# jw007123/hp-Adaptive-Signed-Distance-Field-Octree

Hardware: AMD Instinct MI355X
Metric: Query() Mpts/sec at targetError=1e-5 (union3 field, 10M SplitMix64 pts per GPU, HBM-resident); Create() ms reported as create_ms (higher is better)
Workload: dtype f64

## Files before the change

### hp-adaptive-signed-distance-field-octree_amd/csrc/field_eval.hpp

```cpp
#pragma once
#include <hip/hip_runtime.h>

#include "device_types.hpp"

namespace hpsdf {

template <bool LEFT>
__device__ __forceinline__ double sum3(double a, double b, double c) {
    if constexpr (LEFT) return (a + b) + c;
    else return a + (b + c);
}
template <bool LEFT>
__device__ __forceinline__ double prod3(double a, double b, double c) {
    if constexpr (LEFT) return (a * b) * c;
    else return a * (b * c);
}
__device__ __forceinline__ double sqrtExact(double x) {
    const uint32_t hi = (uint32_t)__double2hiint(x);
    const bool plain = hi - 0x10000000u < 0x7FF00000u - 0x10000000u;
    if (__builtin_amdgcn_ballot_w64(!plain) != 0ull) return sqrt(x);
    const double y = __builtin_amdgcn_rsq(x);
    double g = x * y, h = y * 0.5;
    const double r = __builtin_fma(-h, g, 0.5);
    g = __builtin_fma(g, r, g);
    h = __builtin_fma(h, r, h);
    double d = __builtin_fma(-g, g, x);
    g = __builtin_fma(d, h, g);
    d = __builtin_fma(-g, g, x);
    return __builtin_fma(d, h, g);
}

template <bool LEFT>
__device__ __forceinline__ double norm3(double x, double y, double z) { return sqrtExact(sum3<LEFT>(x * x, y * y, z * z)); }

template <bool LEFT>
__device__ __forceinline__ double primEval(const hpsdf_prim& pr, double x, double y, double z) {
    const double* p = pr.p;
    switch (pr.kind) {
        case HPSDF_PRIM_SPHERE:
            return norm3<LEFT>(x - p[0], y - p[1], z - p[2]) - p[3];
        case HPSDF_PRIM_BOX: {
            const double qx = fabs(x - p[0]) - p[3];
            const double qy = fabs(y - p[1]) - p[4];
            const double qz = fabs(z - p[2]) - p[5];
            const double outside = norm3<LEFT>(fmax(qx, 0.0), fmax(qy, 0.0), fmax(qz, 0.0));
            const double inside = fmin(fmax(qx, fmax(qy, qz)), 0.0);
            return outside + inside;
        }
        case HPSDF_PRIM_TORUS_Y: {
            const double dx = x - p[0], dy = y - p[1], dz = z - p[2];
            const double l = sqrtExact(dx * dx + dz * dz) - p[3];
            return sqrtExact(l * l + dy * dy) - p[4];
        }
        case HPSDF_PRIM_PLANE:
            return (p[0] * x + (p[1] * y + p[2] * z)) + p[3];
        default:
            return 0.0;
    }
}

template <bool LEFT>
__device__ __forceinline__ double analyticEval(const FieldDev& f, double x, double y, double z) {
    double acc = primEval<LEFT>(f.prims[0], x, y, z);
    for (int i = 1; i < f.nPrims; ++i) {
        const double d = primEval<LEFT>(f.prims[i], x, y, z);
        switch (f.prims[i].op) {
            case HPSDF_OP_UNION: acc = fmin(acc, d); break;
            case HPSDF_OP_INTERSECT: acc = fmax(acc, d); break;
            default: acc = fmax(acc, -d); break;
        }
    }
    return acc;
}

}
```

### hp-adaptive-signed-distance-field-octree_amd/csrc/fit_kernels.hpp

```cpp
#pragma once
#include <hip/hip_runtime.h>

#include <cstdint>

#include "device_types.hpp"
#include "field_glue.hpp"
#include "launch.hpp"

namespace hpsdf {


constexpr int kFitPiece = 8;
#ifndef HPSDF_FIT_MIN_WAVES
#define HPSDF_FIT_MIN_WAVES 4
#endif

__device__ __forceinline__ double fitRowAny(double acc, double a1, const double* __restrict__ tk, double n2,
                                            const double* __restrict__ F, int nq) {
    int k = 0;
    for (; k + 4 <= nq; k += 4) {
        const double f0 = F[k], f1 = F[k + 1], f2 = F[k + 2], f3 = F[k + 3];
        const double t0 = tk[k], t1 = tk[k + 1], t2 = tk[k + 2], t3 = tk[k + 3];
        acc = acc + (a1 * t0 * n2) * f0;
        acc = acc + (a1 * t1 * n2) * f1;
        acc = acc + (a1 * t2 * n2) * f2;
        acc = acc + (a1 * t3 * n2) * f3;
    }
    for (; k < nq; ++k) acc = acc + (a1 * tk[k] * n2) * F[k];
    return acc;
}

template <int KIND, bool CSG, int DEG, int R, bool LEFT>
__device__ __forceinline__ void fitBlockBody(const FitBlock blk, const FitTask* __restrict__ tasks, double* __restrict__ arena,
                                             double* __restrict__ errs, double* __restrict__ mirror,
                                             const DeviceTables* __restrict__ T, const FieldDev& field, const RootMap& rm, double* lds) {
    static_assert(R == 1 || DEG > 0, "cell blocking needs a compile-time degree");
    __shared__ double sNl[13 * 11];
    __shared__ double sRec[26];
    __shared__ int32_t sMeshStack[kFitThreads / 64][kMeshStack];
    __shared__ unsigned char sPosI[KIND == kFieldMesh ? 64 : 4], sPosJK[KIND == kFieldMesh ? 64 : 4];
    const int tid = threadIdx.x;
    const int deg = DEG > 0 ? DEG : (int)blk.degree;
    const int nq = 4 * deg + 1, nq2 = nq * nq, G = blk.nTasks;
    const int rowStart = blk.rowStart, rowEnd = blk.rowEnd, nrows = rowEnd - rowStart;
    const int gl = nq * (nq - 1) / 2;
    const int planes = blk.planesPerChunk;
    const int depth = blk.depth;
    const bool split = blk.split != 0;

    double* sT = lds;
    double* sR = sT + (deg + 1) * nq;
    double* sW = sR + nq;
    double* sC = sW + nq;
    double* sF = sC + 8 * G;

    stageQueryTables(T, sNl, sRec);
    for (int q = tid; q < nq; q += kFitThreads) {
        const double x = T->roots[gl + q];
        sR[q] = x;
        sW[q] = T->weights[gl + q];
        double m2 = 0.0, m1 = 1.0;
        sT[q] = 1.0;
        for (int i = 1; i <= deg; ++i) {
            const double l = T->rec[i][0] * x * m1 - T->rec[i][1] * m2;
            m2 = m1, m1 = l;
            sT[i * nq + q] = l;
        }
    }
    for (int g = tid; g < G; g += kFitThreads) {
        const FitTask& tk = tasks[blk.firstTask + g];
        double sc[3];
        for (int a = 0; a < 3; ++a) {
            sc[a] = (double)(tk.bmax[a] - tk.bmin[a]) * 0.5;
            sC[8 * g + 3 + a] = (double)((tk.bmin[a] + tk.bmax[a]) / 2.0f);
            sC[8 * g + a] = sc[a];
        }
        sC[8 * g + 6] = prod3<LEFT>(sc[0], sc[1], sc[2]);
        sC[8 * g + 7] = __longlong_as_double((long long)tk.sampleOff);
    }
    __syncthreads();

    const bool wide = DEG == 0 && nrows > kFitThreads;
    const int slot = wide ? 0 : tid / nrows;
    const int g2 = slot * R;
    const int r0 = rowStart + (wide ? tid : tid % nrows);
    const int r1 = r0 + kFitThreads;
    const bool act0 = wide ? (r0 < rowEnd) : (tid < ((G + R - 1) / R) * nrows);
    const bool act1 = wide && r1 < rowEnd;
    int i0a = 0, i1a = 0, i2a = 0, i0b = 0, i1b = 0, i2b = 0;
    double n0a = 0, n1a = 0, n2a = 0, n0b = 0, n1b = 0, n2b = 0;
    if (act0) {
        i0a = T->bidx[r0][0], i1a = T->bidx[r0][1], i2a = T->bidx[r0][2];
        n0a = sNl[i0a * 11 + depth], n1a = sNl[i1a * 11 + depth], n2a = sNl[i2a * 11 + depth];
    }
    if (act1) {
        i0b = T->bidx[r1][0], i1b = T->bidx[r1][1], i2b = T->bidx[r1][2];
        n0b = sNl[i0b * 11 + depth], n1b = sNl[i1b * 11 + depth], n2b = sNl[i2b * 11 + depth];
    }
    constexpr int NQF = DEG > 0 ? 4 * DEG + 1 : 1;
    double tkReg[NQF];
    if (DEG > 0) {
#pragma unroll
        for (int k = 0; k < NQF; ++k) tkReg[k] = sT[i2a * nq + k];
    }
    uint32_t meshHint = 0xFFFFFFFFu;
    double acc[R];
#pragma unroll
    for (int r = 0; r < R; ++r) acc[r] = 0.0;
    double acc1 = 0.0;

    const int cellStride = planes * nq2;
    for (int iBase = 0; iBase < nq; iBase += planes) {
        const int np = min(planes, nq - iBase);
        if constexpr (KIND == kFieldMesh) {
            if (tid < nq) {
                int rank = 0;
                for (int b = 0; b < nq; ++b) rank += sR[b] < sR[tid] ? 1 : 0;
                sPosJK[rank] = (unsigned char)tid;
            }
            if (tid >= 64 && tid < 64 + np) {
                const int a = tid - 64;
                int rank = 0;
                for (int b = 0; b < np; ++b) rank += sR[iBase + b] < sR[iBase + a] ? 1 : 0;
                sPosI[rank] = (unsigned char)a;
            }
            __syncthreads();
        }
        if constexpr (KIND != kFieldMesh) {
            const int cols = G * nq2;
            for (int c0 = 0; c0 < cols; c0 += kFitThreads) {
                const int cc = c0 + tid;
                const bool activeS = cc < cols;
                const int ccl = activeS ? cc : cols - 1;
                const int g = ccl / nq2, jk = ccl - g * nq2, j = jk / nq, k = jk - j * nq;
                const double* c = sC + 8 * g;
                const double uy = sR[j] * c[1] + c[4], uz = sR[k] * c[2] + c[5];
                const double wy = uy * rm.bounds[1] + rm.centre[1];
                const double wz = uz * rm.bounds[2] + rm.centre[2];
                const double wj = sW[j], wk = sW[k], c6 = c[6];
                const uint64_t sbase = (uint64_t)__double_as_longlong(c[7]) + (uint64_t)(j * nq + k);
                for (int il = 0; il < np; ++il) {
                    const int i = iBase + il;
                    const double ux = sR[i] * c[0] + c[3];
                    const double wx = ux * rm.bounds[0] + rm.centre[0];
                    const uint64_t sidx = sbase + (uint64_t)(i * nq2);
                    const double fv = activeS ? fieldEvalWorld<KIND, CSG, LEFT>(field, wx, wy, wz, sidx, sNl, sRec, meshHint) : 0.0;
                    if (activeS) {
                        sF[g * cellStride + il * nq2 + jk] = c6 * prod3<LEFT>(sW[i], wj, wk) * fv;
                        if (split) const_cast<double*>(field.samples)[sidx] = fv;
                    }
                }
            }
        } else {
            const int chunkSamples = np * nq2, total = G * chunkSamples;
            const float invChunk = 1.0f / (float)chunkSamples;
            for (int s0 = 0; s0 < total; s0 += kFitThreads) {
                const int s = s0 + tid;
                const bool activeS = s < total;
                const int sc = activeS ? s : total - 1;
                int g = (int)(((float)sc + 0.5f) * invChunk);
                int rem = sc - g * chunkSamples;
                if (rem < 0) {
                    --g;
                    rem += chunkSamples;
                } else if (rem >= chunkSamples) {
                    ++g;
                    rem -= chunkSamples;
                }
                if constexpr (KIND == kFieldMesh) rem = meshSampleOrder(rem, np, nq, sPosI, sPosJK);
                const double* c = sC + 8 * g;
                const int il = rem / nq2, jk = rem - il * nq2, j = jk / nq, k = jk - j * nq, i = iBase + il;
                const double ux = sR[i] * c[0] + c[3], uy = sR[j] * c[1] + c[4], uz = sR[k] * c[2] + c[5];
                const double wx = ux * rm.bounds[0] + rm.centre[0];
                const double wy = uy * rm.bounds[1] + rm.centre[1];
                const double wz = uz * rm.bounds[2] + rm.centre[2];
                const uint64_t sidx = (uint64_t)__double_as_longlong(c[7]) + (uint64_t)((i * nq + j) * nq + k);
                double fv;
                if constexpr (KIND == kFieldMesh) {
                    const double mv = (double)meshSignedDistanceWave(field.mesh, V3{(float)wx, (float)wy, (float)wz}, activeS, meshHint,
                                                                     sMeshStack[tid >> 6]);
                    fv = activeS ? applyCsg<CSG>(field, mv, wx, wy, wz, sNl, sRec) : 0.0;
                } else {
                    fv = activeS ? fieldEvalWorld<KIND, CSG, LEFT>(field, wx, wy, wz, sidx, sNl, sRec, meshHint) : 0.0;
                }
                if (activeS) {
                    sF[g * cellStride + rem] = c[6] * prod3<LEFT>(sW[i], sW[j], sW[k]) * fv;
                    if constexpr (KIND != kFieldMesh)
                        if (split) const_cast<double*>(field.samples)[sidx] = fv;
                }
            }
        }
        __syncthreads();
        if (act0) {
            const double* tj = sT + i1a * nq;
            const double* tk = sT + i2a * nq;
            for (int il = 0; il < np; ++il) {
                const double* F = sF + g2 * cellStride + il * nq2;
                const double a0 = sT[i0a * nq + iBase + il] * n0a;
#ifdef HPSDF_FIT_ROW_UNROLL
#pragma unroll HPSDF_FIT_ROW_UNROLL
#endif
                for (int j = 0; j < nq; ++j) {
                    const double a1 = a0 * tj[j] * n1a;
                    if constexpr (DEG > 0 && DEG <= 5) {
                        double lp[NQF];
#pragma unroll
                        for (int k = 0; k < NQF; ++k) lp[k] = a1 * tkReg[k] * n2a;
#pragma unroll
                        for (int r = 0; r < R; ++r) {
                            const double* Fr = F + r * cellStride + j * nq;
                            double f[NQF];
#pragma unroll
                            for (int k = 0; k < NQF; ++k) f[k] = Fr[k];
#pragma unroll
                            for (int k = 0; k < NQF; ++k) acc[r] = acc[r] + lp[k] * f[k];
                        }
                    } else if constexpr (DEG > 5) {
                        const double* Fr = F + j * nq;
#pragma unroll
                        for (int k0 = 0; k0 < NQF; k0 += kFitPiece) {
                            double lp[kFitPiece], f[kFitPiece];
#pragma unroll
                            for (int k = 0; k < kFitPiece; ++k)
                                if (k0 + k < NQF) f[k] = Fr[k0 + k];
#pragma unroll
                            for (int k = 0; k < kFitPiece; ++k)
                                if (k0 + k < NQF) lp[k] = a1 * tkReg[k0 + k] * n2a;
#pragma unroll
                            for (int k = 0; k < kFitPiece; ++k)
                                if (k0 + k < NQF) acc[0] = acc[0] + lp[k] * f[k];
                        }
                    } else {
                        acc[0] = fitRowAny(acc[0], a1, tk, n2a, F + j * nq, nq);
                    }
                }
            }
        }
        if (act1) {
            const double* tj = sT + i1b * nq;
            const double* tk = sT + i2b * nq;
            for (int il = 0; il < np; ++il) {
                const double* F = sF + il * nq2;
                const double a0 = sT[i0b * nq + iBase + il] * n0b;
                for (int j = 0; j < nq; ++j) {
                    const double a1 = a0 * tj[j] * n1b;
                    acc1 = fitRowAny(acc1, a1, tk, n2b, F + j * nq, nq);
                }
            }
        }
        __syncthreads();
    }

    const bool weighted = blk.weighted != 0;
    const int stashStride = weighted ? rowEnd : nrows, stashBase = weighted ? 0 : rowStart;
    const int outBase = split ? 0 : stashBase;
    if (act0) {
#pragma unroll
        for (int r = 0; r < R; ++r)
            if (g2 + r < G) {
                const uint64_t at = tasks[blk.firstTask + g2 + r].outOff + (r0 - outBase);
                arena[at] = acc[r];
                if (mirror != nullptr) mirror[at] = acc[r];
                sF[(g2 + r) * stashStride + (r0 - stashBase)] = acc[r];
            }
    }
    if (act1) {
        arena[tasks[blk.firstTask].outOff + (r1 - outBase)] = acc1;
        sF[r1 - stashBase] = acc1;
    }
    if (weighted && rowStart > 0) {
        for (int s = tid; s < G * rowStart; s += kFitThreads) {
            const int g = s / rowStart, r = s - g * rowStart;
            const FitTask& tk = tasks[blk.firstTask + g];
            const double v = arena[tk.copyOff + r];
            arena[tk.outOff + r] = v;
            sF[g * stashStride + r] = v;
        }
    }
    __syncthreads();
    for (int g = tid; g < G; g += kFitThreads) {
        const int first = deg > 0 ? (int)T->count[deg - 1] : 0;
        double e = 0.0;
        for (int r = first > rowStart ? first : rowStart; r < rowEnd; ++r)
            if (T->bidx[r][3] == deg) {
                const double c = sF[g * stashStride + (r - stashBase)];
                e = e + c * c;
            }
        errs[tasks[blk.firstTask + g].errSlot] = e;
    }
}

template <int KIND, bool CSG, bool LEFT>
__global__ __launch_bounds__(kFitThreads, HPSDF_FIT_MIN_WAVES) void fit_multi_kernel(const FitBlock* __restrict__ blocks,
                                                                const FitTask* __restrict__ tasks, double* __restrict__ arena,
                                                                double* __restrict__ errs, const DeviceTables* __restrict__ T,
                                                                FieldDev field, RootMap rm, const uint32_t* __restrict__ count,
                                                                uint32_t countValue) {
    extern __shared__ double lds[];
    const uint32_t n = count ? *count : countValue;
    if (blockIdx.x >= n) return;
    const FitBlock blk = blocks[n - 1u - blockIdx.x];
    switch (blk.degree) {
        case 2: fitBlockBody<KIND, CSG, 2, 1, LEFT>(blk, tasks, arena, errs, nullptr, T, field, rm, lds); break;
        case 3: fitBlockBody<KIND, CSG, 3, 1, LEFT>(blk, tasks, arena, errs, nullptr, T, field, rm, lds); break;
        case 4: fitBlockBody<KIND, CSG, 4, 1, LEFT>(blk, tasks, arena, errs, nullptr, T, field, rm, lds); break;
        case 5: fitBlockBody<KIND, CSG, 5, 1, LEFT>(blk, tasks, arena, errs, nullptr, T, field, rm, lds); break;
        case 6: fitBlockBody<KIND, CSG, 6, 1, LEFT>(blk, tasks, arena, errs, nullptr, T, field, rm, lds); break;
        case 7: fitBlockBody<KIND, CSG, 7, 1, LEFT>(blk, tasks, arena, errs, nullptr, T, field, rm, lds); break;
        case 8: fitBlockBody<KIND, CSG, 8, 1, LEFT>(blk, tasks, arena, errs, nullptr, T, field, rm, lds); break;
        default: fitBlockBody<KIND, CSG, 0, 1, LEFT>(blk, tasks, arena, errs, nullptr, T, field, rm, lds); break;
    }
}

template <int KIND, bool CSG, int DEG, int R, bool LEFT>
__global__ __launch_bounds__(kFitThreads, HPSDF_FIT_MIN_WAVES) void fit_kernel(const FitBlock* __restrict__ blocks,
                                                          const FitTask* __restrict__ tasks, double* __restrict__ arena,
                                                          double* __restrict__ errs, double* __restrict__ mirror,
                                                          const DeviceTables* __restrict__ T, FieldDev field, RootMap rm,
                                                          const uint32_t* __restrict__ range) {
    extern __shared__ double lds[];
    uint32_t b = blockIdx.x;
    if (range != nullptr) {
        if (b >= range[1]) return;
        b += range[0];
    }
    fitBlockBody<KIND, CSG, DEG, R, LEFT>(blocks[b], tasks, arena, errs, mirror, T, field, rm, lds);
}

template <int KIND, bool CSG, bool LEFT>
__global__ __launch_bounds__(256) void field_kernel(FieldDev f, const DeviceTables* __restrict__ T,
                                                    const double* __restrict__ xyz, size_t n, double* __restrict__ out) {
    __shared__ double sNl[13 * 11];
    __shared__ double sRec[26];
    stageQueryTables(T, sNl, sRec);
    __syncthreads();
    const size_t stride = (size_t)gridDim.x * blockDim.x;
    uint32_t hint = 0xFFFFFFFFu;
    for (size_t i = (size_t)blockIdx.x * blockDim.x + threadIdx.x; i < n; i += stride)
        out[i] = fieldEvalWorld<KIND, CSG, LEFT>(f, xyz[3 * i], xyz[3 * i + 1], xyz[3 * i + 2], i, sNl, sRec, hint);
}

template <int KIND, bool CSG, bool LEFT>
static void launchFitT(hipStream_t stream, int degree, int cellsPerThread, const FitBlock* dBlocks, uint32_t nBlocks,
                       size_t ldsBytes, const FitTask* dTasks, double* dArena, double* dErrs, double* dMeans,
                       const DeviceTables* dTables, const FieldDev& field, const RootMap& rm, const uint32_t* dRange) {
#define HPSDF_FIT_LAUNCH(D, RR)                                                                                       \
    hipLaunchKernelGGL((fit_kernel<KIND, CSG, D, RR, LEFT>), dim3(nBlocks), dim3(kFitThreads), ldsBytes, stream, dBlocks, \
                       dTasks, dArena, dErrs, dMeans, dTables, field, rm, dRange)
#define HPSDF_FIT_CASE(D)       \
    case D:                     \
        HPSDF_FIT_LAUNCH(D, 1); \
        break;
    if (cellsPerThread != 1 && cellsPerThread != 4) cellsPerThread = 1;
    switch (degree) {
        HPSDF_FIT_CASE(2)
        HPSDF_FIT_CASE(3)
        HPSDF_FIT_CASE(4)
        HPSDF_FIT_CASE(5)
        HPSDF_FIT_CASE(6)
        HPSDF_FIT_CASE(7)
        HPSDF_FIT_CASE(8)
        default:
            HPSDF_FIT_LAUNCH(0, 1);
    }
#undef HPSDF_FIT_CASE
#undef HPSDF_FIT_LAUNCH
}

template <int KIND, bool CSG, bool LEFT>
static void launchFitMultiT(hipStream_t stream, const FitBlock* dBlocks, uint32_t maxBlocks, size_t ldsBytes, const FitTask* dTasks,
                            double* dArena, double* dErrs, const DeviceTables* dTables, const FieldDev& field, const RootMap& rm,
                            const uint32_t* dCount) {
    hipLaunchKernelGGL((fit_multi_kernel<KIND, CSG, LEFT>), dim3(maxBlocks), dim3(kFitThreads), ldsBytes, stream, dBlocks, dTasks, dArena, dErrs,
                       dTables, field, rm, dCount, maxBlocks);
}

template <int KIND, bool CSG, bool LEFT>
static void launchFieldT(hipStream_t stream, const FieldDev& f, const DeviceTables* dTables, const double* dXyz,
                         size_t n, double* dOut) {
    hipLaunchKernelGGL((field_kernel<KIND, CSG, LEFT>), dim3(gridFor(n)), dim3(256), 0, stream, f, dTables, dXyz, n, dOut);
}

#define HPSDF_DISPATCH_FIELD_ORDER(FN, K, C, field, ...)  \
    do {                                                  \
        if ((field).leftAssoc) FN<K, C, true>(__VA_ARGS__); \
        else FN<K, C, false>(__VA_ARGS__);                \
    } while (0)
#define HPSDF_DISPATCH_FIELD(FN, K, field, ...)                                                  \
    do {                                                                                         \
        if ((field).csgOp >= 0) HPSDF_DISPATCH_FIELD_ORDER(FN, K, true, field, __VA_ARGS__);     \
        else HPSDF_DISPATCH_FIELD_ORDER(FN, K, false, field, __VA_ARGS__);                       \
    } while (0)

template <int KIND>
void launchFitKind(hipStream_t stream, int degree, int cellsPerThread, const FitBlock* dBlocks, uint32_t nBlocks, size_t ldsBytes,
                   const FitTask* dTasks, double* dArena, double* dErrs, double* dMirror, const DeviceTables* dTables,
                   const FieldDev& field, const RootMap& rm, const uint32_t* dRange) {
    HPSDF_DISPATCH_FIELD(launchFitT, KIND, field, stream, degree, cellsPerThread, dBlocks, nBlocks, ldsBytes, dTasks, dArena,
                         dErrs, dMirror, dTables, field, rm, dRange);
}
template <int KIND>
void launchFitMultiKind(hipStream_t stream, const FitBlock* dBlocks, uint32_t maxBlocks, size_t ldsBytes, const FitTask* dTasks,
                        double* dArena, double* dErrs, const DeviceTables* dTables, const FieldDev& field, const RootMap& rm,
                        const uint32_t* dCount) {
    HPSDF_DISPATCH_FIELD(launchFitMultiT, KIND, field, stream, dBlocks, maxBlocks, ldsBytes, dTasks, dArena, dErrs, dTables, field, rm, dCount);
}
template <int KIND>
void launchFieldKind(hipStream_t stream, const FieldDev& f, const DeviceTables* dTables, const double* dXyz, size_t n, double* dOut) {
    HPSDF_DISPATCH_FIELD(launchFieldT, KIND, f, stream, f, dTables, dXyz, n, dOut);
}
#undef HPSDF_DISPATCH_FIELD
#undef HPSDF_DISPATCH_FIELD_ORDER

#define HPSDF_FIT_KIND_UNIT(EXTERN, K)                                                                                                 \
    EXTERN template void launchFitKind<K>(hipStream_t, int, int, const FitBlock*, uint32_t, size_t, const FitTask*, double*, double*, \
                                          double*, const DeviceTables*, const FieldDev&, const RootMap&, const uint32_t*);            \
    EXTERN template void launchFitMultiKind<K>(hipStream_t, const FitBlock*, uint32_t, size_t, const FitTask*, double*, double*,      \
                                               const DeviceTables*, const FieldDev&, const RootMap&, const uint32_t*);                \
    EXTERN template void launchFieldKind<K>(hipStream_t, const FieldDev&, const DeviceTables*, const double*, size_t, double*);
HPSDF_FIT_KIND_UNIT(extern, kFieldAnalytic)
HPSDF_FIT_KIND_UNIT(extern, kFieldSamples)
HPSDF_FIT_KIND_UNIT(extern, kFieldMesh)

}
```

Before: 92580.

## Evaluate analytic field in y-columns reusing x/z terms in fit kernel

Adds column-wise analytic SDF evaluation that computes the x/z-dependent parts of each primitive once and evaluates N y-samples together, with one wave-level ballot deciding fast or exact sqrt for the whole column. The fit kernel's non-CSG analytic path is remapped so each thread owns an (i,k) column and walks j in pieces, with a degree-dependent piece size. This targets redundant per-sample arithmetic in Create(), at the cost of more register pressure and extra index math. Query throughput is not directly touched.

```diff
diff --git a/hp-adaptive-signed-distance-field-octree_amd/csrc/field_eval.hpp b/hp-adaptive-signed-distance-field-octree_amd/csrc/field_eval.hpp
--- a/hp-adaptive-signed-distance-field-octree_amd/csrc/field_eval.hpp
+++ b/hp-adaptive-signed-distance-field-octree_amd/csrc/field_eval.hpp
@@ -15,10 +15,11 @@
     if constexpr (LEFT) return (a * b) * c;
     else return a * (b * c);
 }
-__device__ __forceinline__ double sqrtExact(double x) {
+__device__ __forceinline__ bool sqrtPlain(double x) {
     const uint32_t hi = (uint32_t)__double2hiint(x);
-    const bool plain = hi - 0x10000000u < 0x7FF00000u - 0x10000000u;
-    if (__builtin_amdgcn_ballot_w64(!plain) != 0ull) return sqrt(x);
+    return hi - 0x10000000u < 0x7FF00000u - 0x10000000u;
+}
+__device__ __forceinline__ double sqrtFast(double x) {
     const double y = __builtin_amdgcn_rsq(x);
     double g = x * y, h = y * 0.5;
     const double r = __builtin_fma(-h, g, 0.5);
@@ -29,33 +30,118 @@
     d = __builtin_fma(-g, g, x);
     return __builtin_fma(d, h, g);
 }
+__device__ __forceinline__ double sqrtExact(double x) {
+    if (__builtin_amdgcn_ballot_w64(!sqrtPlain(x)) != 0ull) return sqrt(x);
+    return sqrtFast(x);
+}
+template <int N>
+__device__ __forceinline__ void sqrtExactColumn(double (&x)[N]) {
+    bool plain = true;
+#pragma unroll
+    for (int s = 0; s < N; ++s) plain = plain && sqrtPlain(x[s]);
+    if (__builtin_amdgcn_ballot_w64(!plain) != 0ull) {
+#pragma unroll
+        for (int s = 0; s < N; ++s) x[s] = sqrt(x[s]);
+    } else {
+#pragma unroll
+        for (int s = 0; s < N; ++s) x[s] = sqrtFast(x[s]);
+    }
+}
 
 template <bool LEFT>
-__device__ __forceinline__ double norm3(double x, double y, double z) { return sqrtExact(sum3<LEFT>(x * x, y * y, z * z)); }
+__device__ __forceinline__ double sphereArg(const double* p, double dx2, double dz2, double y) {
+    const double dy = y - p[1];
+    return sum3<LEFT>(dx2, dy * dy, dz2);
+}
+__device__ __forceinline__ double boxQ(double v, double centre, double half) { return fabs(v - centre) - half; }
+template <bool LEFT>
+__device__ __forceinline__ double boxArg(const double* p, double mx2, double mz2, double y) {
+    const double my = fmax(boxQ(y, p[1], p[4]), 0.0);
+    return sum3<LEFT>(mx2, my * my, mz2);
+}
+__device__ __forceinline__ double boxInside(const double* p, double qx, double qz, double y) {
+    return fmin(fmax(qx, fmax(boxQ(y, p[1], p[4]), qz)), 0.0);
+}
+__device__ __forceinline__ double torusL(const double* p, double x, double z) {
+    const double dx = x - p[0], dz = z - p[2];
+    return sqrtExact(dx * dx + dz * dz) - p[3];
+}
+__device__ __forceinline__ double torusArg(const double* p, double l2, double y) {
+    const double dy = y - p[1];
+    return l2 + dy * dy;
+}
+__device__ __forceinline__ double planeDist(const double* p, double px, double pz, double y) { return (px + (p[1] * y + pz)) + p[3]; }
 
 template <bool LEFT>
 __device__ __forceinline__ double primEval(const hpsdf_prim& pr, double x, double y, double z) {
     const double* p = pr.p;
     switch (pr.kind) {
-        case HPSDF_PRIM_SPHERE:
-            return norm3<LEFT>(x - p[0], y - p[1], z - p[2]) - p[3];
+        case HPSDF_PRIM_SPHERE: {
+            const double dx = x - p[0], dz = z - p[2];
+            return sqrtExact(sphereArg<LEFT>(p, dx * dx, dz * dz, y)) - p[3];
+        }
         case HPSDF_PRIM_BOX: {
-            const double qx = fabs(x - p[0]) - p[3];
-            const double qy = fabs(y - p[1]) - p[4];
-            const double qz = fabs(z - p[2]) - p[5];
-            const double outside = norm3<LEFT>(fmax(qx, 0.0), fmax(qy, 0.0), fmax(qz, 0.0));
-            const double inside = fmin(fmax(qx, fmax(qy, qz)), 0.0);
-            return outside + inside;
+            const double qx = boxQ(x, p[0], p[3]), qz = boxQ(z, p[2], p[5]);
+            const double mx = fmax(qx, 0.0), mz = fmax(qz, 0.0);
+            return sqrtExact(boxArg<LEFT>(p, mx * mx, mz * mz, y)) + boxInside(p, qx, qz, y);
         }
         case HPSDF_PRIM_TORUS_Y: {
-            const double dx = x - p[0], dy = y - p[1], dz = z - p[2];
-            const double l = sqrtExact(dx * dx + dz * dz) - p[3];
-            return sqrtExact(l * l + dy * dy) - p[4];
+            const double l = torusL(p, x, z);
+            return sqrtExact(torusArg(p, l * l, y)) - p[4];
         }
         case HPSDF_PRIM_PLANE:
-            return (p[0] * x + (p[1] * y + p[2] * z)) + p[3];
+            return planeDist(p, p[0] * x, p[2] * z, y);
         default:
             return 0.0;
+    }
+}
+
+template <bool LEFT, int N>
+__device__ __forceinline__ void primEvalColumn(const hpsdf_prim& pr, double x, double z, const double (&y)[N], double (&d)[N]) {
+    const int kind = pr.kind;
+    const double p[6] = {pr.p[0], pr.p[1], pr.p[2], pr.p[3], pr.p[4], pr.p[5]};
+    switch (kind) {
+        case HPSDF_PRIM_SPHERE: {
+            const double dx = x - p[0], dz = z - p[2];
+            const double dx2 = dx * dx, dz2 = dz * dz, r = p[3];
+#pragma unroll
+            for (int s = 0; s < N; ++s) d[s] = sphereArg<LEFT>(p, dx2, dz2, y[s]);
+            sqrtExactColumn<N>(d);
+#pragma unroll
+            for (int s = 0; s < N; ++s) d[s] = d[s] - r;
+            break;
+        }
+        case HPSDF_PRIM_BOX: {
+            const double qx = boxQ(x, p[0], p[3]), qz = boxQ(z, p[2], p[5]);
+            const double mx = fmax(qx, 0.0), mz = fmax(qz, 0.0);
+            const double mx2 = mx * mx, mz2 = mz * mz;
+#pragma unroll
+            for (int s = 0; s < N; ++s) d[s] = boxArg<LEFT>(p, mx2, mz2, y[s]);
+            sqrtExactColumn<N>(d);
+#pragma unroll
+            for (int s = 0; s < N; ++s) d[s] = d[s] + boxInside(p, qx, qz, y[s]);
+            break;
+        }
+        case HPSDF_PRIM_TORUS_Y: {
+            const double l = torusL(p, x, z);
+            const double l2 = l * l, r = p[4];
+#pragma unroll
+            for (int s = 0; s < N; ++s) d[s] = torusArg(p, l2, y[s]);
+            sqrtExactColumn<N>(d);
+#pragma unroll
+            for (int s = 0; s < N; ++s) d[s] = d[s] - r;
+            break;
+        }
+        case HPSDF_PRIM_PLANE: {
+            const double px = p[0] * x, pz = p[2] * z;
+#pragma unroll
+            for (int s = 0; s < N; ++s) d[s] = planeDist(p, px, pz, y[s]);
+            break;
+        }
+        default:
+#pragma unroll
+            for (int s = 0; s < N; ++s) d[s] = 0.0;
+            break;
     }
 }
 
@@ -73,4 +159,28 @@
     return acc;
 }
 
+template <bool LEFT, int N>
+__device__ __forceinline__ void analyticEvalColumn(const FieldDev& f, double x, double z, const double (&y)[N], double (&out)[N]) {
+    primEvalColumn<LEFT, N>(f.prims[0], x, z, y, out);
+    for (int i = 1; i < f.nPrims; ++i) {
+        double d[N];
+        const int op = f.prims[i].op;
+        primEvalColumn<LEFT, N>(f.prims[i], x, z, y, d);
+        switch (op) {
+            case HPSDF_OP_UNION:
+#pragma unroll
+                for (int s = 0; s < N; ++s) out[s] = fmin(out[s], d[s]);
+                break;
+            case HPSDF_OP_INTERSECT:
+#pragma unroll
+                for (int s = 0; s < N; ++s) out[s] = fmax(out[s], d[s]);
+                break;
+            default:
+#pragma unroll
+                for (int s = 0; s < N; ++s) out[s] = fmax(out[s], -d[s]);
+                break;
+        }
+    }
 }
+
+}
diff --git a/hp-adaptive-signed-distance-field-octree_amd/csrc/fit_kernels.hpp b/hp-adaptive-signed-distance-field-octree_amd/csrc/fit_kernels.hpp
--- a/hp-adaptive-signed-distance-field-octree_amd/csrc/fit_kernels.hpp
+++ b/hp-adaptive-signed-distance-field-octree_amd/csrc/fit_kernels.hpp
@@ -2,6 +2,7 @@
 #include <hip/hip_runtime.h>
 
 #include <cstdint>
+#include <type_traits>
 
 #include "device_types.hpp"
 #include "field_glue.hpp"
@@ -11,6 +12,7 @@
 
 
 constexpr int kFitPiece = 8;
+constexpr int fitColumnPiece(int deg) { return deg == 0 ? 2 : deg == 2 ? 3 : deg <= 4 ? 4 : deg == 5 || deg == 8 ? 1 : 2; }
 #ifndef HPSDF_FIT_MIN_WAVES
 #define HPSDF_FIT_MIN_WAVES 4
 #endif
@@ -126,7 +128,61 @@
             }
             __syncthreads();
         }
-        if constexpr (KIND != kFieldMesh) {
+        if constexpr (KIND == kFieldAnalytic && !CSG) {
+            constexpr int N = fitColumnPiece(DEG);
+            const int cellCols = np * nq, cols = G * cellCols;
+            const float invCellCols = 1.0f / (float)cellCols;
+            for (int c0 = 0; c0 < cols; c0 += kFitThreads) {
+                const int cc = c0 + tid;
+                if (cc >= cols) continue;
+                int g = (int)(((float)cc + 0.5f) * invCellCols);
+                int rem = cc - g * cellCols;
+                if (rem < 0) {
+                    --g;
+                    rem += cellCols;
+                } else if (rem >= cellCols) {
+                    ++g;
+                    rem -= cellCols;
+                }
+                const int il = rem / nq, k = rem - il * nq, i = iBase + il;
+                const double* c = sC + 8 * g;
+                const double ux = sR[i] * c[0] + c[3], uz = sR[k] * c[2] + c[5];
+                const double wx = ux * rm.bounds[0] + rm.centre[0];
+                const double wz = uz * rm.bounds[2] + rm.centre[2];
+                double* Fc = sF + g * cellStride + il * nq2 + k;
+                auto piece = [&](int j0, auto size) {
+                    constexpr int M = decltype(size)::value;
+                    double wy[M], fv[M];
+                    const double c1 = c[1], c4 = c[4];
+#pragma unroll
+                    for (int s = 0; s < M; ++s) {
+                        const double uy = sR[DEG > 0 ? j0 + s : min(j0 + s, nq - 1)] * c1 + c4;
+                        wy[s] = uy * rm.bounds[1] + rm.centre[1];
+                    }
+                    double px = wx, pz = wz;
+                    if (M < nq) asm volatile("" : "+v"(px), "+v"(pz));
+                    analyticEvalColumn<LEFT, M>(field, px, pz, wy, fv);
+                    const double wi = sW[i], wk = sW[k], c6 = c[6];
+                    const uint64_t sbase = (uint64_t)__double_as_longlong(c[7]) + (uint64_t)(i * nq2 + k);
+#pragma unroll
+                    for (int s = 0; s < M; ++s) {
+                        const int j = j0 + s;
+                        if (DEG > 0 || j < nq) {
+                            Fc[j * nq] = c6 * prod3<LEFT>(wi, sW[j], wk) * fv[s];
+                            if (split) const_cast<double*>(field.samples)[sbase + (uint64_t)(j * nq)] = fv[s];
+                        }
+                    }
+                };
+                if constexpr (DEG > 0) {
+#pragma unroll 1
+                    for (int j0 = 0; j0 + N <= NQF; j0 += N) piece(j0, std::integral_constant<int, N>());
+                    if constexpr (NQF % N != 0) piece(NQF - NQF % N, std::integral_constant<int, NQF % N>());
+                } else {
+#pragma unroll 1
+                    for (int j0 = 0; j0 < nq; j0 += N) piece(j0, std::integral_constant<int, N>());
+                }
+            }
+        } else if constexpr (KIND != kFieldMesh) {
             const int cols = G * nq2;
             for (int c0 = 0; c0 < cols; c0 += kFitThreads) {
                 const int cc = c0 + tid;
```

Result: no change. 92490 (-0.1%).
